# Dont4rootMe/beast_tokenizer

Measured on AMD Instinct MI355X. Metric: trajectories/sec encode+reconstruct (B=4096,T=50,DoF=14), higher is better.
Workload: dtype f32 (fp32 MFMA fit, int64 tokens); 1 GPU; BEASTBsplineTokenizer encode->reconstruct_traj, num_dof=14 num_basis=10 seq_len=50 vocab=256 degree_p=4; global_batch=4096, per_gpu_batch=4096, seq_len=50, parallelism=dp1

## Files before the change

### beast_tokenizer_amd/csrc/codec.hip

```cpp
#include <hip/hip_runtime.h>

#include <atomic>

#include <algorithm>
#include <cstdlib>

#include "common.h"

namespace {

constexpr int NTHREADS = 256;
constexpr int NWAVES = NTHREADS / 64;
constexpr int MAX_T = 256;
constexpr int MAX_N = 16;
constexpr int MAX_D = 64;
constexpr int ECH = 4;

typedef double double4_t __attribute__((ext_vector_type(4)));
typedef float float4_t __attribute__((ext_vector_type(4)));

__host__ __device__ constexpr int round_up(int x, int m) { return (x + m - 1) / m * m; }

struct FastDiv {
  uint32_t d, m;
// ... 29 lines not shown
}

template <int MAXK>
__device__ __forceinline__ void burst(void* __restrict__ dst, const void* __restrict__ src, int bytes) {
  if (bytes <= 0) return;
  if ((((uintptr_t)src | (uintptr_t)dst) & 15) == 0) {
    const int n16 = bytes >> 4;
    if (n16) burst16<MAXK>(reinterpret_cast<uint4*>(dst), reinterpret_cast<const uint4*>(src), n16);
    const int done = n16 << 4;
    if (done < bytes)
      burst4<1>(reinterpret_cast<uint32_t*>(static_cast<char*>(dst) + done),
                reinterpret_cast<const uint32_t*>(static_cast<const char*>(src) + done), (bytes - done) >> 2);
  } else {
    burst4<4 * MAXK>(reinterpret_cast<uint32_t*>(dst), reinterpret_cast<const uint32_t*>(src), bytes >> 2);
  }
}

#ifndef BEAST_LAT_SP
#define BEAST_LAT_SP 2
#endif
constexpr int LAT_SP = BEAST_LAT_SP;
typedef unsigned u32x4_t __attribute__((ext_vector_type(4)));
template <int SP>
__device__ __forceinline__ void st16(void* p, u32x4_t v) {
  if constexpr (SP == 1) {
    __builtin_nontemporal_store(v, static_cast<u32x4_t*>(p));
  } else if constexpr (SP == 2) {
    asm volatile("global_store_dwordx4 %0, %1, off sc1\n\ts_nop 1" ::"v"(p), "v"(v) : "memory");
  } else {
    *static_cast<u32x4_t*>(p) = v;
  }
}
template <int SP>
__device__ __forceinline__ void st4(float* p, float v) {
  if constexpr (SP == 2) asm volatile("global_store_dword %0, %1, off sc1" ::"v"(p), "v"(v) : "memory");
  else *p = v;
}
template <int SP>
__device__ __forceinline__ void st16(void* p, float4 v) {
  st16<SP>(p, u32x4_t{__float_as_uint(v.x), __float_as_uint(v.y), __float_as_uint(v.z), __float_as_uint(v.w)});
}
template <int SP>
__device__ __forceinline__ void st16(void* p, long long a, long long b) {
  st16<SP>(p, u32x4_t{(unsigned)a, (unsigned)((unsigned long long)a >> 32), (unsigned)b,
                      (unsigned)((unsigned long long)b >> 32)});
}

template <int NT = NTHREADS, int SP = 0>
__device__ __forceinline__ void store_out(float* __restrict__ dst, const float* __restrict__ src, int count) {
  if ((((uintptr_t)src | (uintptr_t)dst) & 15) == 0) {
    const int n4 = count >> 2;
    const float4* s4 = reinterpret_cast<const float4*>(src);
    float4* d4 = reinterpret_cast<float4*>(dst);
    for (int i = threadIdx.x; i < n4; i += NT) st16<SP>(d4 + i, s4[i]);
    for (int i = (n4 << 2) + threadIdx.x; i < count; i += NT) dst[i] = src[i];
  } else {
    for (int i = threadIdx.x; i < count; i += NT) dst[i] = src[i];
  }
}

typedef __attribute__((address_space(3))) void lds_void;

template <int NT = NTHREADS>
__device__ __forceinline__ void dma16(void* lds, const void* g, int n16) {
  const int tid = threadIdx.x, wb = tid & ~63;
  for (int base = 0; base < n16; base += NT) {
    if (base + wb < n16)
      __builtin_amdgcn_global_load_lds(static_cast<const uint4*>(g) + min(base + tid, n16 - 1),
                                       (lds_void*)(static_cast<uint4*>(lds) + base + wb), 16, 0, 0);
  }
}

template <int NT = NTHREADS>
__device__ __forceinline__ void dma4(void* lds, const void* g, int n) {
  const int tid = threadIdx.x, wb = tid & ~63;
  for (int base = 0; base < n; base += NT) {
    if (base + wb < n)
      __builtin_amdgcn_global_load_lds(static_cast<const uint32_t*>(g) + min(base + tid, n - 1),
                                       (lds_void*)(static_cast<uint32_t*>(lds) + base + wb), 4, 0, 0);
  }
}

#ifdef BEAST_STAMPS
__device__ unsigned long long g_stamps[2][8][16];
#define STAMP(k, i)                                                                              \
  do {                                                                                           \
    if (blockIdx.x == 0 && (threadIdx.x & 63) == 0) g_stamps[k][threadIdx.x >> 6][i] = __builtin_amdgcn_s_memtime(); \
  } while (0)
__device__ unsigned long long g_bstamps[2][4096][4];
#define BSTAMP(k, i)                                                                             \
  do {                                                                                           \
    if (threadIdx.x == 0 && blockIdx.x < 4096) {                                                 \
      g_bstamps[k][blockIdx.x][i] = __builtin_amdgcn_s_memrealtime();                            \
      if (i == 0)                                                                                \
        g_bstamps[k][blockIdx.x][2] = ((unsigned long long)__builtin_amdgcn_s_getreg(0xF814) << 32) | \
                                      (unsigned)__builtin_amdgcn_s_getreg(0xF804);               \
    }                                                                                            \
  } while (0)
#else
#define STAMP(k, i) do { } while (0)
#define BSTAMP(k, i) do { } while (0)
#endif

struct Geom {
  int D, nj, N, T, Tp, per;
  int nq0, nq;
  FastDiv fd_nj, fd_ng, fd_per, fd_N, fd_D, fd_nq;
};

template <int TBT>
inline Geom make_geom(int D, int nj, int N, int T) {
  Geom g;
  g.D = D; g.nj = nj; g.N = N; g.T = T; g.Tp = round_up(T, 4); g.per = N * D;
  const int ng = D - nj;
  g.nq0 = (TBT * nj + 15) / 16;
  g.nq = g.nq0 + (TBT * ng + 15) / 16;
  g.fd_nj = make_fd(std::max(nj, 1));
  g.fd_ng = make_fd(std::max(ng, 1));
  g.fd_per = make_fd(g.per);
  g.fd_N = make_fd(N);
  g.fd_D = make_fd(D);
  g.fd_nq = make_fd(std::max(g.nq, 1));
  return g;
}

template <int SD, int SNJ, int SN, int ST, int SDL, int SW = NWAVES>
struct Shape {
  static constexpr int D = SD, NJ = SNJ, N = SN, T = ST, DL = SDL;
  static constexpr int W = SW;
  static constexpr bool fixed = SD > 0;
};
using DynShape = Shape<0, 0, 0, 0, 0>;

template <class S>
struct Dims {
  int D, nj, ng, N, T, Tp, per;
  __device__ __forceinline__ Dims(const Geom& g)
      : D(S::D ? S::D : g.D), nj(S::fixed ? S::NJ : g.nj), ng(D - nj), N(S::N ? S::N : g.N),
        T(S::T ? S::T : g.T), Tp(S::T ? round_up(S::T, 4) : g.Tp), per(N * D) {}
};

template <class S>
__device__ __forceinline__ uint32_t div_by(uint32_t x, int dconst, const FastDiv& f) {
  return S::fixed ? x / (uint32_t)dconst : fdiv(x, f);
}

template <int TBT, class S>
__device__ __forceinline__ void tile_col(const Geom& g, const Dims<S>& m, int q, int lc, int& j, int& d, int& kind,
                                         bool& valid) {
  const int nq0 = (TBT * m.nj + 15) / 16;
  const int k0 = q < nq0 ? 0 : 1;
  const int dk = k0 ? m.ng : m.nj;
  const int c = (q - (k0 ? nq0 : 0)) * 16 + lc;
  valid = c < TBT * dk;
  const uint32_t cc = valid ? c : TBT * dk - 1;
  const uint32_t jj = k0 ? div_by<S>(cc, m.ng > 0 ? m.ng : 1, g.fd_ng) : div_by<S>(cc, m.nj > 0 ? m.nj : 1, g.fd_nj);
  j = (int)jj;
  d = (int)(cc - jj * dk) + (k0 ? m.nj : 0);
  kind = k0;
}

template <int TBT, class S>
__device__ __forceinline__ int n_coltiles(const Dims<S>& m) {
  return (TBT * m.nj + 15) / 16 + (TBT * m.ng + 15) / 16;
}

struct EncArgs {
// ... 179 lines not shown
    if (tile == blockIdx.x) STAMP(0, 4);

    constexpr int SP = (S::W == 7) ? LAT_SP : 0;
    if (a.params_out != nullptr && (a.phases & 4)) store_out<NT, SP>(a.params_out + b0 * DN, pb, nb * DN);
    if (tile == blockIdx.x) STAMP(0, 5);
    if (quant && (a.phases & 8)) {
      const int total = nb * per;
      long long* tout = a.tokens_out + b0 * per;
      const unsigned long long off = (unsigned long long)a.tok_offset;
      auto col_of = [&](int e, int& pj) {
        const int j = (int)div_by<S>((uint32_t)e, per, g.fd_per);
        const int r = e - j * per;
        const int n = (int)div_by<S>((uint32_t)r, D, g.fd_D);
        pj = j * DN;
        return (r - n * D) * N + n;
      };
      int done = 0;
      if ((((uintptr_t)tout) & 15) == 0) {
        const int n4 = total >> 2;
        for (int i = tid; i < n4; i += NT) {
          int bin[4], c[4], pj[4];
          float pv[4];
          float4 qv[4];
          bool ex = false;
#pragma unroll
          for (int u = 0; u < 4; ++u) c[u] = col_of(4 * i + u, pj[u]);
#pragma unroll
          for (int u = 0; u < 4; ++u) { pv[u] = pb[pj[u] + c[u]]; qv[u] = kq[c[u]]; }
#pragma unroll
          for (int u = 0; u < 4; ++u) bin[u] = beast::quantize_bin_k(pv[u], qv[u].x, qv[u].y, qv[u].z, vm1, ex);
          if (ex) {
#pragma unroll
            for (int u = 0; u < 4; ++u) bin[u] = beast::quantize_bin(pv[u], qv[u].x, qv[u].y, vm1);
          }
          st16<SP>(tout + 4 * i, beast::widen_bin(bin[0], off), beast::widen_bin(bin[1], off));
          st16<SP>(tout + 4 * i + 2, beast::widen_bin(bin[2], off), beast::widen_bin(bin[3], off));
        }
        done = n4 << 2;
      }
      for (int e = done + tid; e < total; e += NT) {
        int pj;
        const int c = col_of(e, pj);
        tout[e] = beast::widen_bin(beast::quantize_bin(pb[pj + c], wlo[c], whi[c], vm1), off);
      }
    }
    if (tile == blockIdx.x) STAMP(0, 6);
    if (tile == blockIdx.x + gridDim.x) STAMP(0, 14);
  }
#ifdef BEAST_STAMPS
  __builtin_amdgcn_s_waitcnt(0);
  STAMP(0, 7);
  BSTAMP(0, 1);
#endif
}

template <class S>
struct VShape {
  static_assert(S::fixed && S::T > 0 && S::DL > 0 && ((S::T * S::DL) % 4) == 0, "per-trajectory encode: fixed shape");
  static constexpr int T = S::T, DL = S::DL, D = S::D, N = S::N, DN = S::D * S::N, Tp = round_up(S::T, 4);
  static constexpr int NST = Tp / 4;
};

#ifndef BEAST_RV_WE
#define BEAST_RV_WE 16
#endif
#ifndef BEAST_RV_WR
#define BEAST_RV_WR 16
#endif
constexpr int RV_WE = BEAST_RV_WE, RV_WR = BEAST_RV_WR, RV_WE_BULK = 8;
struct EvSmem {
  int Y, P, wlo, whi, lcol, pimg, timg, total;
};
template <class S, int W>
__host__ __device__ constexpr EvSmem ev_smem(int nkinds) {
  using PS = VShape<S>;
  EvSmem s{};
  int o = 0;
  s.Y = o;    o += round_up(W * PS::T * PS::DL * 4, 1024);
  s.P = o;    o += round_up(nkinds * 16 * PS::Tp * 4, 1024);
  s.wlo = o;  o += round_up(PS::DN * 4, 256);
  s.whi = o;  o += round_up(PS::DN * 4, 256);
  s.lcol = o; o += round_up(PS::D * 4, 256);
  s.pimg = o; o += W * round_up(PS::DN * 4, 16);
  s.timg = o; o += W * round_up(PS::DN * 8, 16);
  s.total = o;
  return s;
}

template <class S, int SP, int W>
__global__ __launch_bounds__(W * 64) void k_encode_v(const float* __restrict__ traj, int64_t B, EncVArgs a) {
  using PS = VShape<S>;
  static_assert(PS::D <= 16 && PS::N <= 16 && PS::DL == PS::D, "per-trajectory encode: D, N <= 16, rows of D");
  constexpr int NT = W * 64, D = PS::D, N = PS::N, T = PS::T, Tp = PS::Tp, DN = PS::DN, NST = PS::NST;
  constexpr int NJ = S::NJ;
  constexpr int nkinds = NJ < D ? 2 : 1;
  constexpr EvSmem L = ev_smem<S, W>(nkinds);
  constexpr int PIMG = round_up(DN * 4, 16) / 4, TIMG = round_up(DN * 8, 16) / 8;
  static_assert((T * D) % 4 == 0 && (DN % 2) == 0, "per-trajectory encode: whole 16-byte rows");
  extern __shared__ __attribute__((aligned(16))) unsigned char smem[];
  float* Y = reinterpret_cast<float*>(smem + L.Y);
  float* P = reinterpret_cast<float*>(smem + L.P);
  float* wlo = reinterpret_cast<float*>(smem + L.wlo);
  float* whi = reinterpret_cast<float*>(smem + L.whi);
  int* lcol = reinterpret_cast<int*>(smem + L.lcol);
  const int tid = threadIdx.x, wave = __builtin_amdgcn_readfirstlane(tid >> 6), lane = tid & 63;
  const int64_t b0 = (int64_t)blockIdx.x * W;
  const int nb = (int)min<int64_t>(W, B - b0);
  const bool quant = a.tokens_out != nullptr;
  STAMP(0, 0);
  BSTAMP(0, 0);
  constexpr int tile16 = T * D / 4;
  dma16<NT>(Y, reinterpret_cast<const float4*>(traj) + b0 * tile16, nb * tile16);
  STAMP(0, 9);
  dma16<NT>(P, a.proj, nkinds * 4 * Tp);
  if (quant) {
    dma4<NT>(wlo, a.w_min, DN);
    dma4<NT>(whi, a.w_max, DN);
  }
  dma4<NT>(lcol, a.dof_src, D);
  const float vm1 = (float)(a.vocab - 1);
  __syncthreads();
  STAMP(0, 2);
  const int j = wave;
  if (j >= nb) return;
  const int lr = lane & 15, lk = lane >> 4;
  const bool dok = lr < D;
  const int c = dok ? min(max(lcol[lr], 0), D - 1) : 0;
  const float* yc = Y + j * T * D + c;
  float4_t acc0 = {0.0f, 0.0f, 0.0f, 0.0f}, acc1 = acc0;
#pragma unroll
  for (int kd = 0; kd < nkinds; ++kd) {
    const bool mine = dok && (nkinds == 1 || ((lr < NJ) == (kd == 0)));
    const float* pa = P + (kd * 16 + lr) * Tp + lk;
    float xa[NST], ya[NST];
#pragma unroll
    for (int st = 0; st < NST; ++st) {
      xa[st] = pa[4 * st];
      const float y = yc[min(4 * st + lk, T - 1) * D];
      ya[st] = mine ? y : 0.0f;
    }
#pragma unroll
    for (int st = 0; st < NST; ++st) {
      if (st & 1) acc1 = __builtin_amdgcn_mfma_f32_16x16x4f32(xa[st], ya[st], acc1, 0, 0, 0);
      else acc0 = __builtin_amdgcn_mfma_f32_16x16x4f32(xa[st], ya[st], acc0, 0, 0, 0);
    }
  }
  STAMP(0, 3);
  float* pimg = reinterpret_cast<float*>(smem + L.pimg) + j * PIMG;
  long long* timg = reinterpret_cast<long long*>(smem + L.timg) + j * TIMG;
  float pv[4];
#pragma unroll
  for (int r = 0; r < 4; ++r) pv[r] = __fadd_rn(acc0[r], acc1[r]);
  if (dok) {
    float* q = pimg + lr * N + 4 * lk;
#pragma unroll
    for (int r = 0; r < 4; r += 2) {
      if (4 * lk + r + 1 < N) *reinterpret_cast<float2*>(q + r) = make_float2(pv[r], pv[r + 1]);
      else if (4 * lk + r < N) q[r] = pv[r];
    }
  }
  if (quant) {
    const unsigned long long off = (unsigned long long)a.tok_offset;
    float lo[4], hi[4];
#pragma unroll
    for (int r = 0; r < 4; ++r) {
      const int k = lr * N + min(4 * lk + r, N - 1);
      lo[r] = wlo[min(k, DN - 1)];
      hi[r] = whi[min(k, DN - 1)];
    }
    int bin[4];
    bool ex = false;
#pragma unroll
    for (int r = 0; r < 4; ++r)
      bin[r] = beast::quantize_bin_k(pv[r], lo[r], hi[r], beast::quantize_scale(lo[r], hi[r], vm1), vm1, ex);
    if (ex) {
#pragma unroll
      for (int r = 0; r < 4; ++r) bin[r] = beast::quantize_bin(pv[r], lo[r], hi[r], vm1);
    }
    if (dok) {
#pragma unroll
      for (int r = 0; r < 4; ++r)
        if (4 * lk + r < N) timg[(4 * lk + r) * D + lr] = beast::widen_bin(bin[r], off);
    }
  }
  __builtin_amdgcn_fence(__ATOMIC_RELEASE, "wavefront");
  __builtin_amdgcn_wave_barrier();
  __builtin_amdgcn_fence(__ATOMIC_ACQUIRE, "wavefront");
  STAMP(0, 5);
  if (a.phases & 4) {
    if (a.params_out != nullptr) {
      float4* gp = reinterpret_cast<float4*>(a.params_out + (b0 + j) * DN);
#pragma unroll
      for (int u = 0; u < (DN / 4 + 63) / 64; ++u) {
        const int i = u * 64 + lane;
        if (i < DN / 4) st16<SP>(gp + i, reinterpret_cast<const float4*>(pimg)[i]);
      }
    }
    if (quant) {
      long long* gt = a.tokens_out + (b0 + j) * DN;
#pragma unroll
      for (int u = 0; u < (DN / 2 + 63) / 64; ++u) {
        const int i = u * 64 + lane;
        if (i < DN / 2) st16<SP>(gt + 2 * i, timg[2 * i], timg[2 * i + 1]);
      }
    }
  }
  STAMP(0, 7);
#ifdef BEAST_STAMPS
  __builtin_amdgcn_s_waitcnt(0);
  STAMP(0, 8);
  BSTAMP(0, 1);
#endif
}

struct RecArgs {
  const long long* tokens;
  const float* ntokens;
  int64_t B, ntiles, tok_offset, basis_sb, init_p_sb;
  int vocab, Tout, ndo, phases, lut_n, tbt;
  const float* w_min;
  const float* w_max;
  const float* basis;
  const int32_t* dof_dst;
  const float* init_p;
  const int32_t* init_p_src;
  float* params_out;
  float* pos_out;
  Geom g;
  FastDiv fd_row;
};

struct RecVArgs {
  const float* w_min;
  const float* w_max;
  const float* basis;
  const int32_t* dof_dst;
  const float* init_p;
  const int32_t* init_p_src;
  float* pos_out;
  int64_t tok_offset, init_p_sb;
  int vocab, lut_n, phases;
};

constexpr int LUT_MAX = 4096;
constexpr int RT_REG = 4;

template <int NT = NTHREADS>
__device__ __forceinline__ void stage_rows(void* lds, const void* base, int64_t B, int esz, int64_t b0, int per,
                                           int tbt) {
  const int nb = (int)min<int64_t>(B - b0, tbt);
  const char* src = static_cast<const char*>(base) + b0 * per * esz;
  const int bytes = nb * per * esz;
  if ((bytes & 15) == 0 && (((uintptr_t)src) & 15) == 0) dma16<NT>(lds, src, bytes >> 4);
  else dma4<NT>(lds, src, bytes >> 2);
}

template <int NT = NTHREADS>
__device__ __forceinline__ void stage_tokens(const RecArgs& a, void* lds, int64_t b0, int per) {
  const int nb = (int)min<int64_t>(a.B - b0, a.tbt);
  const void* src = a.ntokens ? static_cast<const void*>(a.ntokens + b0 * per)
                              : static_cast<const void*>(a.tokens + b0 * per);
  const int bytes = nb * per * (a.ntokens ? 4 : 8);
  if ((bytes & 15) == 0 && (((uintptr_t)src) & 15) == 0) dma16<NT>(lds, src, bytes >> 4);
  else dma4<NT>(lds, src, bytes >> 2);
}
// ... 184 lines not shown
      if (tile == blockIdx.x) {
#pragma unroll
        for (int kd = 0; kd < 2; ++kd)
#pragma unroll
          for (int rt = 0; rt < RT; ++rt)
#pragma unroll
            for (int ks = 0; ks < KS; ++ks) {
              const int t = rt * 16 + lr, n = lk * KS + ks;
              const float x = phi[(min(kd, nkinds - 1) * Tout + min(t, Tout - 1)) * N + min(n, N - 1)];
              phr[kd][rt][ks] = (t < Tout && n < N && kd < nkinds) ? x : 0.0f;
            }
      }
    }
    if (a.params_out != nullptr) rec_params_out<NT>(a, tokl, b0, nb, wlo, whi, lut, vm1);

    for (int q = wave; (a.phases & 2) && q < nq; q += NW) {
      int j, d, kind;
      bool ok;
      tile_col<TBT>(g, m, q, lr, j, d, kind, ok);
      ok = ok && j < nb;
      float w[KS];
      rec_weights<KS>(a, tokl, j, d, lk, N, D, per, wlo, whi, lut, vm1, w);
#pragma unroll
      for (int ks = 0; ks < KS; ++ks) w[ks] = (ok && lk * KS + ks < N) ? w[ks] : 0.0f;
      if (a.init_p != nullptr && lk == 0 && ok && d < nj)
        w[0] = a.init_p[(b0 + j) * a.init_p_sb + a.init_p_src[d]];
      float* oc = ob + (j * RTR + lk * 4) * ndo + min(max(dst[d], 0), ndo - 1);
      if constexpr (RT > 0) {
        float4_t acc[RT];
#pragma unroll
        for (int i = 0; i < RT; ++i) acc[i] = float4_t{0.0f, 0.0f, 0.0f, 0.0f};
#pragma unroll
        for (int ks = 0; ks < KS; ++ks)
#pragma unroll
          for (int i = 0; i < RT; ++i)
            acc[i] = __builtin_amdgcn_mfma_f32_16x16x4f32(kind ? phr[1][i][ks] : phr[0][i][ks], w[ks], acc[i], 0,
                                                          0, 0);
        if (ok) {
#pragma unroll
          for (int i = 0; i < RT; ++i)
#pragma unroll
            for (int r = 0; r < 4; ++r) oc[(i * 16 + r) * ndo] = acc[i][r];
        }
      } else {
        const float* Ph = phi + (kind * RTR + lr) * Np4 + lk * KS;
        for (int rt = 0; rt < RTR / 16; rt += 4) {
          float av[4][KS];
#pragma unroll
          for (int i = 0; i < 4; ++i)
#pragma unroll
            for (int ks = 0; ks < KS; ++ks) av[i][ks] = Ph[((rt + i) * 16) * Np4 + ks];
          float4_t acc[4];
#pragma unroll
          for (int i = 0; i < 4; ++i) acc[i] = float4_t{0.0f, 0.0f, 0.0f, 0.0f};
#pragma unroll
          for (int ks = 0; ks < KS; ++ks)
#pragma unroll
            for (int i = 0; i < 4; ++i)
              acc[i] = __builtin_amdgcn_mfma_f32_16x16x4f32(av[i][ks], w[ks], acc[i], 0, 0, 0);
          if (ok) {
#pragma unroll
            for (int i = 0; i < 4; ++i)
#pragma unroll
              for (int r = 0; r < 4; ++r) oc[((rt + i) * 16 + r) * ndo] = acc[i][r];
          }
        }
      }
    }
    if (tile == blockIdx.x) STAMP(1, 5);
    __syncthreads();
    if (tile == blockIdx.x) STAMP(1, 6);
    if (a.phases & 4) rec_store<S>(a, a.pos_out + b0 * (int64_t)Tout * ndo, ob, nb, RTR);
    if (tile == blockIdx.x) STAMP(1, 7);
  }
#ifdef BEAST_STAMPS
  __builtin_amdgcn_s_waitcnt(0);
  STAMP(1, 8);
  BSTAMP(1, 1);
#endif
}


struct RvSmem {
  int tok, wlo, whi, dst, phi, lut, wimg, img, total;
};
template <class S>
__host__ __device__ constexpr RvSmem rv_smem(int nkinds) {
  RvSmem s{};
  constexpr int per = S::D * S::N;
  int o = 0;
  s.tok = o;  o += round_up(RV_WR * per * 8, 1024);
  s.wlo = o;  o += round_up(per * 4, 256);
  s.whi = o;  o += round_up(per * 4, 256);
  s.dst = o;  o += round_up(S::D * 4, 256);
  s.phi = o;  o += round_up(nkinds * S::T * S::N * 4, 1024);
  s.lut = o;  o += round_up(LUT_MAX * 4, 16);
  s.wimg = o; o += round_up(RV_WR * per * 4, 16);
  s.img = o;  o += RV_WR * round_up(S::T * S::D * 4, 16);
  s.total = o;
  return s;
}

template <int KS, class S, int SP>
__global__ __launch_bounds__(RV_WR * 64) void k_reconstruct_v(const void* __restrict__ tsrc, int64_t B, int esz,
                                                             RecVArgs a) {
  static_assert(S::fixed && S::T > 0 && S::T <= 64 && S::D <= 16 && S::DL == S::D && 4 * KS >= S::N,
                "per-trajectory reconstruct: fixed shape, T <= 64, D <= 16, ndo == D");
  constexpr int NT = RV_WR * 64, D = S::D, N = S::N, T = S::T, per = D * N;
  constexpr int NJ = S::NJ;
  constexpr int nkinds = NJ < D ? 2 : 1;
  constexpr RvSmem L = rv_smem<S>(nkinds);
  constexpr int RV_IMG = round_up(T * D * 4, 16) / 4;
  static_assert((T * D) % 4 == 0, "per-trajectory reconstruct: whole 16-byte rows");
  extern __shared__ __attribute__((aligned(16))) unsigned char smem[];
  const unsigned char* tokl = smem + L.tok;
  float* wlo = reinterpret_cast<float*>(smem + L.wlo);
  float* whi = reinterpret_cast<float*>(smem + L.whi);
  int* dst = reinterpret_cast<int*>(smem + L.dst);
  float* phi = reinterpret_cast<float*>(smem + L.phi);
  float* lut = reinterpret_cast<float*>(smem + L.lut);
  const int tid = threadIdx.x, wave = __builtin_amdgcn_readfirstlane(tid >> 6), lane = tid & 63;
  const int64_t b0 = (int64_t)blockIdx.x * RV_WR;
  STAMP(1, 0);
  BSTAMP(1, 0);
  stage_rows<NT>(smem + L.tok, tsrc, B, esz, b0, per, RV_WR);
  STAMP(1, 9);
  dma4<NT>(wlo, a.w_min, per);
  dma4<NT>(whi, a.w_max, per);
  dma4<NT>(dst, a.dof_dst, D);
  {
    constexpr int pbytes = nkinds * T * N * 4;
    if ((pbytes & 15) == 0 && (((uintptr_t)a.basis) & 15) == 0) dma16<NT>(phi, a.basis, pbytes >> 4);
    else dma4<NT>(phi, a.basis, pbytes >> 2);
  }
  const float vm1 = (float)(a.vocab - 1);
  for (int t = tid; t < a.lut_n; t += NT) lut[t] = __fdiv_rn((float)t, vm1);
  STAMP(1, 12);
  __syncthreads();
  STAMP(1, 2);
  const int j = wave;
  const int nb = (int)min<int64_t>(RV_WR, B - b0);
  if (j >= nb) return;
  float* wimg = reinterpret_cast<float*>(smem + L.wimg) + j * per;
  const long long* tk = reinterpret_cast<const long long*>(tokl) + j * per;
#pragma unroll
  for (int u = 0; u < (per + 63) / 64; ++u) {
    const int e = u * 64 + lane;
    if (e < per) {
      const int n = e / D, d = e - n * D, k = d * N + n;
      const float lo = wlo[k], hi = whi[k];
      const long long t = tk[e] - a.tok_offset;
      const float nrm = (t >= 0 && t < a.lut_n) ? lut[(int)t] : __fdiv_rn((float)t, vm1);
      float w = beast::clamp_t(__fadd_rn(__fmul_rn(nrm, __fsub_rn(hi, lo)), lo), lo, hi);
      if (a.init_p != nullptr && n == 0 && d < NJ) w = a.init_p[(b0 + j) * a.init_p_sb + a.init_p_src[d]];
      wimg[k] = w;
    }
  }
  __builtin_amdgcn_fence(__ATOMIC_RELEASE, "wavefront");
  __builtin_amdgcn_wave_barrier();
  __builtin_amdgcn_fence(__ATOMIC_ACQUIRE, "wavefront");
  STAMP(1, 3);
  const int c = lane & 15, kk = lane >> 4;
  int dsrc = -1;
#pragma unroll
  for (int d = 0; d < D; ++d) dsrc = dst[d] == c ? d : dsrc;
  const bool row_ok = dsrc >= 0;
  const int dd = row_ok ? dsrc : 0;
  float av[KS];
#pragma unroll
  for (int s2 = 0; s2 < KS; ++s2) {
    const int n = kk * KS + s2;
    const float w = wimg[dd * N + min(n, N - 1)];
    av[s2] = (row_ok && n < N) ? w : 0.0f;
  }
  float4_t acc[4];
#pragma unroll
  for (int tt = 0; tt < 4; ++tt) acc[tt] = float4_t{0.0f, 0.0f, 0.0f, 0.0f};
#pragma unroll
  for (int kd = 0; kd < nkinds; ++kd) {
    float bv[4][KS];
#pragma unroll
    for (int tt = 0; tt < 4; ++tt)
#pragma unroll
      for (int s2 = 0; s2 < KS; ++s2) {
        const int t = tt * 16 + c, n = kk * KS + s2;
        const float x = phi[(kd * T + min(t, T - 1)) * N + min(n, N - 1)];
        bv[tt][s2] = (t < T && n < N) ? x : 0.0f;
      }
    const bool mine = nkinds == 1 || ((dd < NJ) == (kd == 0));
#pragma unroll
    for (int s2 = 0; s2 < KS; ++s2) {
      const float ak = mine ? av[s2] : 0.0f;
#pragma unroll
      for (int tt = 0; tt < 4; ++tt)
        if (tt * 16 < T) acc[tt] = __builtin_amdgcn_mfma_f32_16x16x4f32(ak, bv[tt][s2], acc[tt], 0, 0, 0);
    }
  }
  STAMP(1, 5);
  float* img = reinterpret_cast<float*>(smem + L.img) + j * RV_IMG;
#pragma unroll
  for (int tt = 0; tt < 4; ++tt) {
    const int t = tt * 16 + c;
    if (tt * 16 < T && t < T) {
      float* q = img + t * D + 4 * kk;
      if (4 * kk + 1 < D) *reinterpret_cast<float2*>(q) = make_float2(acc[tt][0], acc[tt][1]);
      else if (4 * kk < D) q[0] = acc[tt][0];
      if (4 * kk + 3 < D) *reinterpret_cast<float2*>(q + 2) = make_float2(acc[tt][2], acc[tt][3]);
      else if (4 * kk + 2 < D) q[2] = acc[tt][2];
    }
  }
  __builtin_amdgcn_fence(__ATOMIC_RELEASE, "wavefront");
  __builtin_amdgcn_wave_barrier();
  __builtin_amdgcn_fence(__ATOMIC_ACQUIRE, "wavefront");
  STAMP(1, 6);
  if (a.phases & 4) {
    constexpr int n4 = T * D / 4;
    float4* gout = reinterpret_cast<float4*>(a.pos_out + (b0 + j) * (int64_t)T * D);
#pragma unroll
    for (int u = 0; u < (n4 + 63) / 64; ++u) {
      const int i = u * 64 + lane;
      if (i < n4) st16<SP>(gout + i, reinterpret_cast<const float4*>(img)[i]);
    }
  }
  STAMP(1, 7);
#ifdef BEAST_STAMPS
  __builtin_amdgcn_s_waitcnt(0);
  STAMP(1, 8);
  BSTAMP(1, 1);
#endif
}

template <int TBT>
__global__ __launch_bounds__(NTHREADS) void k_reconstruct_rows(RecArgs a) {
  extern __shared__ __attribute__((aligned(16))) unsigned char smem[];
  const Geom& g = a.g;
  const int D = g.D, N = g.N, nj = g.nj, per = g.per;
  const int Tout = a.Tout, ndo = a.ndo;
  const bool pos = a.pos_out != nullptr;
  const RecSmem L = rec_smem<TBT, 0, 0>(Tout, D, N, ndo, (nj < D) ? 2 : 1, a.lut_n);
  const int Np4 = L.Np4;
  const unsigned char* tokl = smem + L.tok;
  float* pb = reinterpret_cast<float*>(smem + L.pb);
  float* wlo = reinterpret_cast<float*>(smem + L.wlo);
  float* whi = reinterpret_cast<float*>(smem + L.whi);
  float* lut = reinterpret_cast<float*>(smem + L.lut);
  uint16_t* pmap = reinterpret_cast<uint16_t*>(smem + L.pmap);
  int* dst = reinterpret_cast<int*>(smem + L.dst);
  int* col2d = reinterpret_cast<int*>(smem + L.col2d);
  float* ob = reinterpret_cast<float*>(smem + L.out);
  const int tid = threadIdx.x;
  const float vm1 = (float)(a.vocab - 1);

  if (blockIdx.x < a.ntiles) stage_tokens(a, smem + L.tok, (int64_t)blockIdx.x * TBT, per);
  dma4(wlo, a.w_min, per);
  dma4(whi, a.w_max, per);
  if (pos) dma4(dst, a.dof_dst, D);
  for (int t = tid; t < a.lut_n; t += NTHREADS) lut[t] = __fdiv_rn((float)t, vm1);
  for (int r = tid; r < per; r += NTHREADS) {
    const int n = r / D, d = r - n * D;
    pmap[r] = (uint16_t)(d * Np4 + n);
  }
  if (pos) {
    __syncthreads();
    for (int c = tid; c < ndo; c += NTHREADS) col2d[c] = -1;
    __syncthreads();
    if (tid < D) {
      const int dd = dst[tid];
      if (dd >= 0 && dd < ndo) col2d[dd] = tid;
    }
  }

  for (int64_t tile = blockIdx.x; tile < a.ntiles; tile += gridDim.x) {
    const int64_t b0 = tile * TBT;
    const int nb = (int)min<int64_t>(TBT, a.B - b0);
    if (tile != blockIdx.x) stage_tokens(a, smem + L.tok, b0, per);
    __syncthreads();
    if (a.params_out != nullptr) rec_params_out(a, tokl, b0, nb, wlo, whi, lut, vm1);
    if (!pos) continue;
    for (int e = tid; e < nb * per; e += NTHREADS) {
      const uint32_t j = fdiv(e, g.fd_per);
      const int r = e - j * per;
      const uint32_t n = fdiv(r, g.fd_D);
      const int d = r - n * D;
      pb[j * D * Np4 + pmap[r]] = rec_weight(a, tokl, e, d * N + n, wlo, whi, lut, vm1);
    }
    __syncthreads();
    if (a.init_p != nullptr) {
// ... 393 lines not shown
```

Baseline: 436.6 million trajectories/s.

## Precompute LDS addresses before barrier and trim quantiser and reconstruct address math

```diff
diff --git a/beast_tokenizer_amd/csrc/codec.hip b/beast_tokenizer_amd/csrc/codec.hip
--- a/beast_tokenizer_amd/csrc/codec.hip
+++ b/beast_tokenizer_amd/csrc/codec.hip
@@ -135,7 +135,7 @@
 }
 
 #ifdef BEAST_STAMPS
-__device__ unsigned long long g_stamps[2][8][16];
+__device__ unsigned long long g_stamps[2][16][16];
 #define STAMP(k, i)                                                                              \
   do {                                                                                           \
     if (blockIdx.x == 0 && (threadIdx.x & 63) == 0) g_stamps[k][threadIdx.x >> 6][i] = __builtin_amdgcn_s_memtime(); \
@@ -481,20 +481,27 @@
   s.whi = o;  o += round_up(PS::DN * 4, 256);
   s.lcol = o; o += round_up(PS::D * 4, 256);
   s.pimg = o; o += W * round_up(PS::DN * 4, 16);
-  s.timg = o; o += W * round_up(PS::DN * 8, 16);
+  s.timg = o; o += W * round_up(PS::DN * 8 + 8, 16);
   s.total = o;
   return s;
+}
+
+template <class V>
+__device__ __forceinline__ void pin(V& v) {
+  asm volatile("" : "+v"(v));
 }
 
 template <class S, int SP, int W>
 __global__ __launch_bounds__(W * 64) void k_encode_v(const float* __restrict__ traj, int64_t B, EncVArgs a) {
   using PS = VShape<S>;
-  static_assert(PS::D <= 16 && PS::N <= 16 && PS::DL == PS::D, "per-trajectory encode: D, N <= 16, rows of D");
+  static_assert(PS::D <= 16 && PS::N <= 10 && PS::DL == PS::D,
+                "per-trajectory encode: D <= 16, rows of D, N <= 10 (three quantiser slots per lane)");
   constexpr int NT = W * 64, D = PS::D, N = PS::N, T = PS::T, Tp = PS::Tp, DN = PS::DN, NST = PS::NST;
   constexpr int NJ = S::NJ;
   constexpr int nkinds = NJ < D ? 2 : 1;
   constexpr EvSmem L = ev_smem<S, W>(nkinds);
-  constexpr int PIMG = round_up(DN * 4, 16) / 4, TIMG = round_up(DN * 8, 16) / 8;
+  constexpr int PIMG = round_up(DN * 4, 16) / 4, TIMG = round_up(DN * 8 + 8, 16) / 8;
+  constexpr int NQ = 3;
   static_assert((T * D) % 4 == 0 && (DN % 2) == 0, "per-trajectory encode: whole 16-byte rows");
   extern __shared__ __attribute__((aligned(16))) unsigned char smem[];
   float* Y = reinterpret_cast<float*>(smem + L.Y);
@@ -517,25 +524,46 @@
     dma4<NT>(whi, a.w_max, DN);
   }
   dma4<NT>(lcol, a.dof_src, D);
+  const int j = wave;
+  const int lr = lane & 15, lk = lane >> 4;
+  const bool dok = lr < D;
   const float vm1 = (float)(a.vocab - 1);
+  int tq[NQ];
+  int kq[NQ];
+#pragma unroll
+  for (int u = 0; u < NQ; ++u) {
+    const int n = (u < 2 || lk < 2) ? 4 * lk + u : 4 * (lk - 2) + 3;
+    kq[u] = (min(lr, D - 1) * N + min(n, N - 1)) * 4;
+    tq[u] = L.timg + (j * TIMG + ((dok && n < N) ? n * D + lr : DN)) * 8;
+    pin(kq[u]); pin(tq[u]);
+  }
+  int yb = L.Y + (j * T * D + lk * D) * 4;
+  int yt = yb + (min(4 * (NST - 1) + lk, T - 1) - lk) * D * 4;
+  int pb = L.P + (lr * Tp + lk) * 4;
+  pin(yb); pin(yt); pin(pb);
   __syncthreads();
   STAMP(0, 2);
-  const int j = wave;
   if (j >= nb) return;
-  const int lr = lane & 15, lk = lane >> 4;
-  const bool dok = lr < D;
-  const int c = dok ? min(max(lcol[lr], 0), D - 1) : 0;
-  const float* yc = Y + j * T * D + c;
+  const int c4 = min(max(lcol[lr], 0), D - 1) * 4;
+  yb += c4;
+  yt += c4;
+  float qlo[NQ] = {0.0f, 0.0f, 0.0f}, qhi[NQ] = {0.0f, 0.0f, 0.0f};
+  if (quant) {
+#pragma unroll
+    for (int u = 0; u < NQ; ++u) {
+      qlo[u] = *reinterpret_cast<const float*>(smem + L.wlo + kq[u]);
+      qhi[u] = *reinterpret_cast<const float*>(smem + L.whi + kq[u]);
+    }
+  }
   float4_t acc0 = {0.0f, 0.0f, 0.0f, 0.0f}, acc1 = acc0;
 #pragma unroll
   for (int kd = 0; kd < nkinds; ++kd) {
-    const bool mine = dok && (nkinds == 1 || ((lr < NJ) == (kd == 0)));
-    const float* pa = P + (kd * 16 + lr) * Tp + lk;
+    const bool mine = nkinds == 1 || (dok && ((lr < NJ) == (kd == 0)));
     float xa[NST], ya[NST];
 #pragma unroll
     for (int st = 0; st < NST; ++st) {
-      xa[st] = pa[4 * st];
-      const float y = yc[min(4 * st + lk, T - 1) * D];
+      xa[st] = *reinterpret_cast<const float*>(smem + pb + (kd * 16 * Tp + 4 * st) * 4);
+      const float y = *reinterpret_cast<const float*>(smem + (st + 1 < NST ? yb + 4 * st * D * 4 : yt));
       ya[st] = mine ? y : 0.0f;
     }
 #pragma unroll
@@ -546,7 +574,7 @@
   }
   STAMP(0, 3);
   float* pimg = reinterpret_cast<float*>(smem + L.pimg) + j * PIMG;
-  long long* timg = reinterpret_cast<long long*>(smem + L.timg) + j * TIMG;
+  const long long* timg = reinterpret_cast<const long long*>(smem + L.timg) + j * TIMG;
   float pv[4];
 #pragma unroll
   for (int r = 0; r < 4; ++r) pv[r] = __fadd_rn(acc0[r], acc1[r]);
@@ -559,27 +587,24 @@
     }
   }
   if (quant) {
-    const unsigned long long off = (unsigned long long)a.tok_offset;
-    float lo[4], hi[4];
-#pragma unroll
-    for (int r = 0; r < 4; ++r) {
-      const int k = lr * N + min(4 * lk + r, N - 1);
-      lo[r] = wlo[min(k, DN - 1)];
-      hi[r] = whi[min(k, DN - 1)];
-    }
-    int bin[4];
+    const auto sw = __builtin_amdgcn_permlane32_swap(__float_as_uint(pv[2]), __float_as_uint(pv[3]), false, false);
+    const float qv[NQ] = {pv[0], pv[1], __uint_as_float(sw[0])};
+    int bin[NQ];
     bool ex = false;
 #pragma unroll
-    for (int r = 0; r < 4; ++r)
-      bin[r] = beast::quantize_bin_k(pv[r], lo[r], hi[r], beast::quantize_scale(lo[r], hi[r], vm1), vm1, ex);
+    for (int u = 0; u < NQ; ++u)
+      bin[u] = beast::quantize_bin_k(qv[u], qlo[u], qhi[u], beast::quantize_scale(qlo[u], qhi[u], vm1), vm1, ex);
     if (ex) {
 #pragma unroll
-      for (int r = 0; r < 4; ++r) bin[r] = beast::quantize_bin(pv[r], lo[r], hi[r], vm1);
-    }
-    if (dok) {
-#pragma unroll
-      for (int r = 0; r < 4; ++r)
-        if (4 * lk + r < N) timg[(4 * lk + r) * D + lr] = beast::widen_bin(bin[r], off);
+      for (int u = 0; u < NQ; ++u) bin[u] = beast::quantize_bin(qv[u], qlo[u], qhi[u], vm1);
+    }
+    if (a.tok_offset == 0) {
+#pragma unroll
+      for (int u = 0; u < NQ; ++u) *reinterpret_cast<long long*>(smem + tq[u]) = beast::widen_bin(bin[u], 0ull);
+    } else {
+      const unsigned long long off = (unsigned long long)a.tok_offset;
+#pragma unroll
+      for (int u = 0; u < NQ; ++u) *reinterpret_cast<long long*>(smem + tq[u]) = beast::widen_bin(bin[u], off);
     }
   }
   __builtin_amdgcn_fence(__ATOMIC_RELEASE, "wavefront");
@@ -930,8 +955,12 @@
 
 
 struct RvSmem {
-  int tok, wlo, whi, dst, phi, lut, wimg, img, total;
+  int tok, wlo, whi, phi, zero, lut, wimg, img, total;
 };
+template <class S>
+__host__ __device__ constexpr int rv_zero_bytes(int nkinds) {
+  return round_up(((nkinds - 1) * S::T + round_up(S::T, 16)) * S::N * 4, 16);
+}
 template <class S>
 __host__ __device__ constexpr RvSmem rv_smem(int nkinds) {
   RvSmem s{};
@@ -940,14 +969,16 @@
   s.tok = o;  o += round_up(RV_WR * per * 8, 1024);
   s.wlo = o;  o += round_up(per * 4, 256);
   s.whi = o;  o += round_up(per * 4, 256);
-  s.dst = o;  o += round_up(S::D * 4, 256);
   s.phi = o;  o += round_up(nkinds * S::T * S::N * 4, 1024);
+  s.zero = o; o += rv_zero_bytes<S>(nkinds);
   s.lut = o;  o += round_up(LUT_MAX * 4, 16);
-  s.wimg = o; o += round_up(RV_WR * per * 4, 16);
+  s.wimg = o; o += round_up(RV_WR * (per + 4) * 4, 16);
   s.img = o;  o += RV_WR * round_up(S::T * S::D * 4, 16);
   s.total = o;
   return s;
 }
+
+typedef __attribute__((address_space(4))) const int32_t const_i32;
 
 template <int KS, class S, int SP>
 __global__ __launch_bounds__(RV_WR * 64) void k_reconstruct_v(const void* __restrict__ tsrc, int64_t B, int esz,
@@ -959,12 +990,13 @@
   constexpr int nkinds = NJ < D ? 2 : 1;
   constexpr RvSmem L = rv_smem<S>(nkinds);
   constexpr int RV_IMG = round_up(T * D * 4, 16) / 4;
+  constexpr int WIMG = per + 4;
+  constexpr int NU = (per + 63) / 64;
+  constexpr int NTT = (T + 15) / 16;
   static_assert((T * D) % 4 == 0, "per-trajectory reconstruct: whole 16-byte rows");
   extern __shared__ __attribute__((aligned(16))) unsigned char smem[];
-  const unsigned char* tokl = smem + L.tok;
   float* wlo = reinterpret_cast<float*>(smem + L.wlo);
   float* whi = reinterpret_cast<float*>(smem + L.whi);
-  int* dst = reinterpret_cast<int*>(smem + L.dst);
   float* phi = reinterpret_cast<float*>(smem + L.phi);
   float* lut = reinterpret_cast<float*>(smem + L.lut);
   const int tid = threadIdx.x, wave = __builtin_amdgcn_readfirstlane(tid >> 6), lane = tid & 63;
@@ -975,7 +1007,6 @@
   STAMP(1, 9);
   dma4<NT>(wlo, a.w_min, per);
   dma4<NT>(whi, a.w_max, per);
-  dma4<NT>(dst, a.dof_dst, D);
   {
     constexpr int pbytes = nkinds * T * N * 4;
     if ((pbytes & 15) == 0 && (((uintptr_t)a.basis) & 15) == 0) dma16<NT>(phi, a.basis, pbytes >> 4);
@@ -983,74 +1014,115 @@
   }
   const float vm1 = (float)(a.vocab - 1);
   for (int t = tid; t < a.lut_n; t += NT) lut[t] = __fdiv_rn((float)t, vm1);
+  for (int i = tid; i < rv_zero_bytes<S>(nkinds) / 4; i += NT) reinterpret_cast<float*>(smem + L.zero)[i] = 0.0f;
   STAMP(1, 12);
+  const int j = wave;
+  const int nb = (int)min<int64_t>(RV_WR, B - b0);
+  int te[NU], kb[NU], wk[NU];
+#pragma unroll
+  for (int u = 0; u < NU; ++u) {
+    const int e = u * 64 + lane, ec = min(e, per - 1);
+    const int n = ec / D, d = ec - n * D, k = d * N + n;
+    te[u] = L.tok + (j * per + ec) * 8;
+    kb[u] = k * 4;
+    wk[u] = L.wimg + (j * WIMG + (e < per ? k : per)) * 4;
+    pin(te[u]); pin(kb[u]); pin(wk[u]);
+  }
+  const int c = lane & 15, kk = lane >> 4;
+  int dsrc = -1;
+  const_i32* dof_dst = (const_i32*)a.dof_dst;
+#pragma unroll
+  for (int d = 0; d < D; ++d) dsrc = dof_dst[d] == c ? d : dsrc;
+  const bool row_ok = dsrc >= 0;
+  const int dd = row_ok ? dsrc : 0;
+  int wa[KS];
+  unsigned am[nkinds];
+#pragma unroll
+  for (int s2 = 0; s2 < KS; ++s2) {
+    const int n = kk * KS + s2;
+    wa[s2] = (row_ok && n < N) ? L.wimg + (j * WIMG + dd * N + n) * 4 : L.zero;
+    pin(wa[s2]);
+  }
+#pragma unroll
+  for (int kd = 0; kd < nkinds; ++kd) {
+    am[kd] = (nkinds == 1 || ((dd < NJ) == (kd == 0))) ? ~0u : 0u;
+    pin(am[kd]);
+  }
+  int pa[KS], pt[KS];
+#pragma unroll
+  for (int s2 = 0; s2 < KS; ++s2) {
+    const int n = kk * KS + s2, tl = (NTT - 1) * 16 + c;
+    pa[s2] = n < N ? L.phi + (c * N + n) * 4 : L.zero;
+    pt[s2] = (n < N && tl < T) ? L.phi + (c * N + n) * 4 : L.zero;
+    pin(pa[s2]); pin(pt[s2]);
+  }
+  int ia = L.img + (j * RV_IMG + c * D + 4 * kk) * 4;
+  pin(ia);
   __syncthreads();
   STAMP(1, 2);
-  const int j = wave;
-  const int nb = (int)min<int64_t>(RV_WR, B - b0);
   if (j >= nb) return;
-  float* wimg = reinterpret_cast<float*>(smem + L.wimg) + j * per;
-  const long long* tk = reinterpret_cast<const long long*>(tokl) + j * per;
-#pragma unroll
-  for (int u = 0; u < (per + 63) / 64; ++u) {
-    const int e = u * 64 + lane;
-    if (e < per) {
-      const int n = e / D, d = e - n * D, k = d * N + n;
-      const float lo = wlo[k], hi = whi[k];
-      const long long t = tk[e] - a.tok_offset;
-      const float nrm = (t >= 0 && t < a.lut_n) ? lut[(int)t] : __fdiv_rn((float)t, vm1);
-      float w = beast::clamp_t(__fadd_rn(__fmul_rn(nrm, __fsub_rn(hi, lo)), lo), lo, hi);
-      if (a.init_p != nullptr && n == 0 && d < NJ) w = a.init_p[(b0 + j) * a.init_p_sb + a.init_p_src[d]];
-      wimg[k] = w;
-    }
+  long long tv[NU];
+  float lo[NU], hi[NU];
+#pragma unroll
+  for (int u = 0; u < NU; ++u) {
+    tv[u] = *reinterpret_cast<const long long*>(smem + te[u]) - a.tok_offset;
+    lo[u] = *reinterpret_cast<const float*>(smem + L.wlo + kb[u]);
+    hi[u] = *reinterpret_cast<const float*>(smem + L.whi + kb[u]);
+  }
+  float nrm[NU];
+  bool far = false;
+#pragma unroll
+  for (int u = 0; u < NU; ++u) {
+    const bool in = (unsigned long long)tv[u] < (unsigned long long)a.lut_n;
+    far = far | !in;
+    nrm[u] = lut[in ? (int)tv[u] : 0];
+  }
+  if (far) {
+#pragma unroll
+    for (int u = 0; u < NU; ++u)
+      if (!((unsigned long long)tv[u] < (unsigned long long)a.lut_n)) nrm[u] = __fdiv_rn((float)tv[u], vm1);
+  }
+#pragma unroll
+  for (int u = 0; u < NU; ++u) {
+    float w = beast::clamp_t(__fadd_rn(__fmul_rn(nrm[u], __fsub_rn(hi[u], lo[u])), lo[u]), lo[u], hi[u]);
+    if (u == 0 && a.init_p != nullptr && lane < NJ)
+      w = a.init_p[(b0 + j) * a.init_p_sb + a.init_p_src[lane]];
+    *reinterpret_cast<float*>(smem + wk[u]) = w;
   }
   __builtin_amdgcn_fence(__ATOMIC_RELEASE, "wavefront");
   __builtin_amdgcn_wave_barrier();
   __builtin_amdgcn_fence(__ATOMIC_ACQUIRE, "wavefront");
   STAMP(1, 3);
-  const int c = lane & 15, kk = lane >> 4;
-  int dsrc = -1;
-#pragma unroll
-  for (int d = 0; d < D; ++d) dsrc = dst[d] == c ? d : dsrc;
-  const bool row_ok = dsrc >= 0;
-  const int dd = row_ok ? dsrc : 0;
-  float av[KS];
-#pragma unroll
-  for (int s2 = 0; s2 < KS; ++s2) {
-    const int n = kk * KS + s2;
-    const float w = wimg[dd * N + min(n, N - 1)];
-    av[s2] = (row_ok && n < N) ? w : 0.0f;
-  }
-  float4_t acc[4];
-#pragma unroll
-  for (int tt = 0; tt < 4; ++tt) acc[tt] = float4_t{0.0f, 0.0f, 0.0f, 0.0f};
+  float4_t acc[NTT];
+#pragma unroll
+  for (int tt = 0; tt < NTT; ++tt) acc[tt] = float4_t{0.0f, 0.0f, 0.0f, 0.0f};
+  float wv[KS];
+#pragma unroll
+  for (int s2 = 0; s2 < KS; ++s2) wv[s2] = *reinterpret_cast<const float*>(smem + wa[s2]);
 #pragma unroll
   for (int kd = 0; kd < nkinds; ++kd) {
-    float bv[4][KS];
-#pragma unroll
-    for (int tt = 0; tt < 4; ++tt)
-#pragma unroll
-      for (int s2 = 0; s2 < KS; ++s2) {
-        const int t = tt * 16 + c, n = kk * KS + s2;
-        const float x = phi[(kd * T + min(t, T - 1)) * N + min(n, N - 1)];
-        bv[tt][s2] = (t < T && n < N) ? x : 0.0f;
-      }
-    const bool mine = nkinds == 1 || ((dd < NJ) == (kd == 0));
+    float bv[NTT][KS];
+#pragma unroll
+    for (int tt = 0; tt < NTT; ++tt)
+#pragma unroll
+      for (int s2 = 0; s2 < KS; ++s2)
+        bv[tt][s2] = *reinterpret_cast<const float*>(smem + (tt * 16 + 15 < T ? pa[s2] : pt[s2]) +
+                                                     (kd * T + tt * 16) * N * 4);
 #pragma unroll
     for (int s2 = 0; s2 < KS; ++s2) {
-      const float ak = mine ? av[s2] : 0.0f;
-#pragma unroll
-      for (int tt = 0; tt < 4; ++tt)
-        if (tt * 16 < T) acc[tt] = __builtin_amdgcn_mfma_f32_16x16x4f32(ak, bv[tt][s2], acc[tt], 0, 0, 0);
+      const float ak = nkinds == 1 ? wv[s2] : __uint_as_float(__float_as_uint(wv[s2]) & am[kd]);
+#pragma unroll
+      for (int tt = 0; tt < NTT; ++tt)
+        acc[tt] = __builtin_amdgcn_mfma_f32_16x16x4f32(ak, bv[tt][s2], acc[tt], 0, 0, 0);
     }
   }
   STAMP(1, 5);
   float* img = reinterpret_cast<float*>(smem + L.img) + j * RV_IMG;
 #pragma unroll
-  for (int tt = 0; tt < 4; ++tt) {
+  for (int tt = 0; tt < NTT; ++tt) {
     const int t = tt * 16 + c;
-    if (tt * 16 < T && t < T) {
-      float* q = img + t * D + 4 * kk;
+    if (t < T) {
+      float* q = reinterpret_cast<float*>(smem + ia + tt * 16 * D * 4);
       if (4 * kk + 1 < D) *reinterpret_cast<float2*>(q) = make_float2(acc[tt][0], acc[tt][1]);
       else if (4 * kk < D) q[0] = acc[tt][0];
       if (4 * kk + 3 < D) *reinterpret_cast<float2*>(q + 2) = make_float2(acc[tt][2], acc[tt][3]);
```

Result: faster. 462.1 million trajectories/s (median of 6 runs) (+5.8%).
